# fpgasystems/gcow

Measured on AMD Instinct MI355X. Metric: GiB/s device-resident fp32->ZFP encode, 256Mi-float bucket, 1/2/4/8 GPU, higher is better.
Workload: dtype f32; 1 GPU; c2_1d_fp32_fixed_rate16_256Mi_per_gpu; layout=1-D contiguous, 4-value blocks, mode=fixed-rate, minbits=64, maxbits=64, bucket_bytes_total=1073741824, launcher=none

## Files before the change

### gcow_amd/csrc/enc_fixed1d.hip

```cpp
#include <hip/hip_runtime.h>

#include <algorithm>
#include <stdint.h>

#include "codec_device.h"
#include "field_io.h"
#include "kernels.h"
#include "lean1d.h"
#include "pipe.h"

#ifndef GCOW_C2_U
#define GCOW_C2_U 8
#endif

namespace gcow {

template <int DT>
__device__ __forceinline__ void load_block1d(const void* in, uint64_t nvals, uint32_t b, float* f)
{
  const uint64_t i0 = 4ull * b;
  if (i0 + 4 <= nvals) {
    load_row4<DT>(in, (int64_t)i0, f);
  } else {
    const uint32_t nv = (uint32_t)(nvals - i0);
#pragma unroll
    for (int x = 0; x < 4; x++) f[x] = load_elem<DT>(in, (int64_t)(i0 + pad_index(x, nv)));
  }
}

__device__ __forceinline__ uint32_t spread2_16(uint32_t x)
{
  x = (x | (x << 8)) & 0x00FF00FFu;
  x = (x | (x << 4)) & 0x0F0F0F0Fu;
  x = (x | (x << 2)) & 0x33333333u;
  x = (x | (x << 1)) & 0x55555555u;
  return x;
}

__device__ __forceinline__ uint64_t interleave4_16(uint32_t a, uint32_t b, uint32_t c, uint32_t d)
{
  const uint32_t P = spread2_16(a) | (spread2_16(c) << 1);
  const uint32_t Q = spread2_16(b) | (spread2_16(d) << 1);
  const uint32_t lo = spread2_16(P & 0xffffu) | (spread2_16(Q & 0xffffu) << 1);
  const uint32_t hi = spread2_16(P >> 16) | (spread2_16(Q >> 16) << 1);
  return (uint64_t)lo | ((uint64_t)hi << 32);
}

template <uint32_t WB>
__device__ __forceinline__ uint64_t encode_block1d_fixed(const float* f, const Params& p, const uint16_t* tab)
{
  float fa[4] = {f[0], f[1], f[2], f[3]};
  const int emax = block_emax<4>(fa);
  const uint32_t prec = precision(emax, p.maxprec, p.minexp, 1);
  if (!prec || emax == -127) return 0ull;
  const float s = cast_scale(emax);
  int32_t q[4];
#pragma unroll
  for (int i = 0; i < 4; i++) q[i] = cast1(fa[i], s);
  fwd_lift(q[0], q[1], q[2], q[3]);
  uint32_t u[4];
#pragma unroll
  for (int i = 0; i < 4; i++) u[i] = ((uint32_t)q[i] + 0xaaaaaaaau) ^ 0xaaaaaaaau;
  const int kmin = prec < 32 ? 32 - (int)prec : 0;
  uint64_t acc = 2ull * (uint32_t)(emax + 127) + 1ull;
  uint32_t pos = 9;
  {
    const int L0 = 31 - (int)__builtin_clz(u[0] | 1u) - (u[0] ? 0 : 1);
    const int L1 = 31 - (int)__builtin_clz(u[1] | 1u) - (u[1] ? 0 : 1);
    const int L2 = 31 - (int)__builtin_clz(u[2] | 1u) - (u[2] ? 0 : 1);
    const int L3 = 31 - (int)__builtin_clz(u[3] | 1u) - (u[3] ? 0 : 1);
    const int M0 = max(max(L0, L1), max(L2, L3));
    const int top = max(M0, kmin - 1);
    pos += (uint32_t)(31 - top);
    uint32_t n = 0;
    const int glo = max(L3, kmin);
    for (int k = top; k >= glo && pos < WB; --k) {
      const uint32_t x = ((u[0] >> k) & 1u) | (((u[1] >> k) & 1u) << 1) | (((u[2] >> k) & 1u) << 2) |
                         (((u[3] >> k) & 1u) << 3);
      const uint32_t e = tab[(n << 4) | x];
      acc |= (uint64_t)(e & 127u) << pos;
      pos += (e >> 7) & 7u;
      n = e >> 10;
    }
    const int kt = L3 - 1;
    if (pos < WB && kt >= kmin) {
      const uint32_t sh = (uint32_t)(31 - kt);
      const uint32_t g0 = __builtin_bitreverse32(u[0]) >> sh, g1 = __builtin_bitreverse32(u[1]) >> sh;
      const uint32_t g2 = __builtin_bitreverse32(u[2]) >> sh, g3 = __builtin_bitreverse32(u[3]) >> sh;
      uint64_t J = interleave4_16(g0 & 0xffffu, g1 & 0xffffu, g2 & 0xffffu, g3 & 0xffffu);
      const uint32_t cnt = (uint32_t)(kt - kmin + 1);
      if (cnt < 16) J &= (1ull << (4 * cnt)) - 1ull;
      acc |= J << pos;
    }
  }
  return WB == 64 ? acc : (acc & ((1ull << WB) - 1ull));
}

template <uint32_t WB, bool W2LOW = false>
__device__ __forceinline__ uint64_t encode_block1d_lean6(const float* f, const uint32_t* tab, const uint32_t* rs,
                                                         bool& special)
{
  uint32_t m;
  asm("v_max3_f32 %0, |%1|, |%2|, |%3|" : "=v"(m) : "v"(f[0]), "v"(f[1]), "v"(f[2]));
  asm("v_max_f32_e64 %0, %0, |%1|" : "+v"(m) : "v"(f[3]));
  special = m >= 0x7f800000u || __builtin_isunordered(f[0], f[1]) || __builtin_isunordered(f[2], f[3]);
  const uint32_t E = m >> 23;
  const float s = __uint_as_float((283u - E) << 23);
  uint32_t x = (uint32_t)cvt_i32_hw(f[0] * s), y = (uint32_t)cvt_i32_hw(f[1] * s);
  uint32_t z = (uint32_t)cvt_i32_hw(f[2] * s), w = (uint32_t)cvt_i32_hw(f[3] * s);
  auto asr = [](uint32_t v) { return (uint32_t)((int32_t)v >> 1); };
  constexpr uint32_t NB = 0xaaaaaaaau;
  x = asr(x + w); w -= x;
  z = asr(z + y); y -= z;
  x = asr(x + z); z -= x;
  w = asr(w + y); y -= w;
  const uint32_t u3 = (w + asr(y) + NB) ^ NB;
  const uint32_t u1 = (y - asr(w + asr(y)) + NB) ^ NB;
  const uint32_t u0 = (x + NB) ^ NB, u2 = (z + NB) ^ NB;
  const uint32_t o23 = u2 | u3;
  const uint32_t sh = __builtin_clz(u0 | u1 | o23 | 1u);
  const int M0 = 31 - (int)sh;
  const int jg = (int)min(ffbh_hw(o23), 31u) - (int)sh;
  const uint32_t w0 = u0 << sh, w1 = u1 << sh, w2 = u2 << sh, w3 = u3 << sh;
  const uint64_t Y = window_lds(rs, w0, w1, w2, w3);
  uint32_t pos = 9 + sh;
  uint32_t e = tab[(uint32_t)Y & 255u];
  uint32_t G = e >> 17, gl = (e >> 13) & 15u;
  int j = 4;
  e = tab5_next(tab, e, ((uint32_t)Y >> 8) & 255u);
  G |= (e >> 17) << gl;
  gl += (e >> 13) & 15u;
  const uint32_t hdr = m ? 2u * E + 3u : 0u;
  uint64_t acc = (uint64_t)hdr | ((uint64_t)G << pos);
  pos += gl;
#pragma unroll
  for (int jj = 4; jj < 16; jj += 2) {
    if (j < jj || !__any(jj <= jg)) break;
    e = tab5_next(tab, e, (uint32_t)(Y >> (4 * jj)) & 255u);
    const uint32_t code = pos < WB ? (e >> 17) : 0u;
    acc |= (uint64_t)code << pos;
    pos += (e >> 13) & 15u;
    j = jj + 2;
  }
  const bool tiny = m - 1u < (29u << 23) - 1u;
  special = special || (!tiny && jg >= 16 && pos < WB);
  if (j < 16 && pos < WB) acc |= (Y >> (4 * j)) << pos;
  const uint32_t p2 = pos + 4u * (uint32_t)(16 - j);
  if (__any(p2 < WB && M0 >= 16)) {
    uint64_t Y2;
    if constexpr (W2LOW) {
      Y2 = window_lds_low(rs, w0, w1, w2, w3);
    } else {
      const uint32_t s2 = sh + 16u;
      Y2 = window_lds(rs, u0 << s2, u1 << s2, u2 << s2, u3 << s2);
    }
    if (p2 < WB && M0 >= 16) acc |= Y2 << p2;
  }
  constexpr uint64_t TINY = tiny_payload_cx((int)WB - 9) << 9;
  acc = tiny ? (TINY | hdr) : acc;
  return WB == 64 ? acc : (acc & ((1ull << WB) - 1ull));
}

template <int DT, uint32_t WB, int U, uint32_t T = 256, int V = 0>
__global__ __launch_bounds__(T) void k_encode_fixed1d_np(const void* __restrict__ in, uint32_t nfull, Params p,
                                                         void* __restrict__ out)
{
  __shared__ __attribute__((aligned(16))) uint32_t tab[1280 + 1024];
  constexpr uint32_t IB = DT == DT_BF16 ? 8u : 16u;
  const pipe_v4i rin = buf_rsrc(in, nfull * IB), rout = buf_rsrc(out, nfull * (WB / 8));
  const uint32_t b0 = blockIdx.x * (T * U) + threadIdx.x;
  typename PipeRow<DT>::T r[U];
  if constexpr ((V & 1) != 0) {
    static_assert(T == 256, "table fill assumes 256 threads");
    constexpr int NT = 1280 / 256;
    const pipe_v4i rt = buf_rsrc(&g_plane_tab5, sizeof(PlaneTab2));
    uint32_t tv[NT];
#pragma unroll
    for (int i = 0; i < NT; i++) tv[i] = buf_load_u32((threadIdx.x + 256u * i) * 4u, rt);
#pragma unroll
    for (int k = 0; k < U; k++) r[k] = PipeRow<DT>::load((b0 + T * k) * IB, rin);
#pragma unroll
    for (uint32_t t = threadIdx.x; t < 1024; t += T) tab[1280 + t] = rspread_entry(t);
    asm volatile("s_waitcnt vmcnt(%5)" : "+v"(tv[0]), "+v"(tv[1]), "+v"(tv[2]), "+v"(tv[3]), "+v"(tv[4]) : "n"(U)
                 : "memory");
#pragma unroll
    for (int i = 0; i < NT; i++) tab[threadIdx.x + 256u * i] = tv[i];
  } else {
#pragma unroll
    for (int k = 0; k < U; k++) r[k] = PipeRow<DT>::load((b0 + T * k) * IB, rin);
#pragma unroll
    for (uint32_t t = threadIdx.x; t < 1280; t += T) tab[t] = g_plane_tab5.v[t];
#pragma unroll
    for (uint32_t t = threadIdx.x; t < 1024; t += T) tab[1280 + t] = rspread_entry(t);
  }
  __syncthreads();
#pragma unroll
  for (int k = 0; k < U; k++) {
    pipe_wait<U - 1>(r[k]);
    float f[4];
    PipeRow<DT>::unpack(r[k], f);
    bool special;
    uint64_t w = encode_block1d_lean6<WB, (V & 2) != 0>(f, tab, tab + 1280, special);
    if (special) {
      RegWriter64 rw{0ull, 0u};
      encode_block<1>(rw, f, p);
      w = WB == 64 ? rw.acc : (rw.acc & ((1ull << WB) - 1ull));
    }
    pipe_store<WB>((b0 + T * k) * (WB / 8), rout, w);
  }
}

template <int DT, uint32_t WB, int U>
__global__ __launch_bounds__(256) void k_copy_pattern1d(const void* __restrict__ in, uint32_t nfull,
                                                        void* __restrict__ out)
{
  constexpr uint32_t T = 256;
  constexpr uint32_t IB = DT == DT_BF16 ? 8u : 16u;
  const pipe_v4i rin = buf_rsrc(in, nfull * IB), rout = buf_rsrc(out, nfull * (WB / 8));
  const uint32_t b0 = blockIdx.x * (T * U) + threadIdx.x;
  typename PipeRow<DT>::T r[U];
#pragma unroll
  for (int k = 0; k < U; k++) r[k] = PipeRow<DT>::load((b0 + T * k) * IB, rin);
#pragma unroll
  for (int k = 0; k < U; k++) {
    pipe_wait<U - 1>(r[k]);
    float f[4];
    PipeRow<DT>::unpack(r[k], f);
    const uint64_t w = ((uint64_t)(__float_as_uint(f[0]) ^ __float_as_uint(f[1])) << 32) |
                       (__float_as_uint(f[2]) ^ __float_as_uint(f[3]));
    pipe_store<WB>((b0 + T * k) * (WB / 8), rout, w);
  }
}

template <int DT, uint32_t WB>
__global__ __launch_bounds__(256) void k_encode_fixed1d_generic(const void* __restrict__ in, uint32_t nfull, Params p,
                                                                void* __restrict__ out)
{
  __shared__ uint16_t tab[80];
  if (threadIdx.x < 80) tab[threadIdx.x] = plane_entry4(threadIdx.x);
  __syncthreads();
  constexpr int U = 2;
  const uint32_t b0 = blockIdx.x * (256u * U) + threadIdx.x;
  float f[U][4];
#pragma unroll
  for (int j = 0; j < U; j++) {
    const uint32_t b = b0 + 256u * j;
    if (b < nfull) load_row4<DT>(in, 4ll * b, f[j]);
  }
#pragma unroll
  for (int j = 0; j < U; j++) {
    const uint32_t b = b0 + 256u * j;
    if (b < nfull) {
      const uint64_t w = encode_block1d_fixed<WB>(f[j], p, tab);
      if constexpr (WB == 64) ((uint64_t*)out)[b] = w;
      else ((uint32_t*)out)[b] = (uint32_t)w;
    }
  }
}

template <int DT, uint32_t WB>
__global__ void k_encode_fixed1d_tail(const void* __restrict__ in, uint64_t nvals, uint32_t b, Params p,
                                      void* __restrict__ out)
{
  __shared__ uint16_t tab[80];
  if (threadIdx.x < 80) tab[threadIdx.x] = plane_entry4(threadIdx.x);
  __syncthreads();
  if (threadIdx.x) return;
  float f[4];
  load_block1d<DT>(in, nvals, b, f);
  const uint64_t w = encode_block1d_fixed<WB>(f, p, tab);
  if constexpr (WB == 64) ((uint64_t*)out)[b] = w;
  else ((uint32_t*)out)[b] = (uint32_t)w;
}

static inline hipStream_t S(void* s) { return (hipStream_t)s; }

template <int DT, uint32_t WB>
static void launch_fixed1d_t(const void* in, uint64_t nvals, const Params& p, void* out, hipStream_t st)
{
  const uint32_t nfull = (uint32_t)(nvals / 4);
  if (nfull) {
    const bool kmin0 = p.maxprec >= 32 && p.minexp <= -154;
    if (!kmin0) {
      k_encode_fixed1d_generic<DT, WB><<<(nfull + 511) / 512, 256, 0, st>>>(in, nfull, p, out);
    } else {
      constexpr uint32_t CH = 1u << 27;
      constexpr uint32_t IB = DT == DT_BF16 ? 8u : 16u;
      for (uint32_t c0 = 0; c0 < nfull; c0 += CH) {
        const uint32_t nc = min(CH, nfull - c0);
        const void* ic = (const char*)in + (size_t)c0 * IB;
        void* oc = (char*)out + (size_t)c0 * (WB / 8);
        constexpr int U = GCOW_C2_U;
        k_encode_fixed1d_np<DT, WB, U, 256, 3><<<(nc + 256 * U - 1) / (256 * U), 256, 0, st>>>(ic, nc, p, oc);
      }
    }
  }
  if (nvals % 4) k_encode_fixed1d_tail<DT, WB><<<1, 128, 0, st>>>(in, nvals, nfull, p, out);
}

hipError_t launch_copy_pattern1d(const void* in, int dtype, uint64_t nvals, uint32_t wb, void* out, void* stream)
{
  const uint32_t nfull = (uint32_t)(nvals / 4);
  constexpr uint32_t CH = 1u << 27;
  const uint32_t IB = dtype == DT_BF16 ? 8u : 16u;
  for (uint32_t c0 = 0; c0 < nfull; c0 += CH) {
    const uint32_t nc = std::min(CH, nfull - c0);
    const void* ic = (const char*)in + (size_t)c0 * IB;
    void* oc = (char*)out + (size_t)c0 * (wb / 8);
    const uint32_t g = (nc + 2047) / 2048;
    if (dtype == DT_BF16) {
      if (wb == 64) k_copy_pattern1d<DT_BF16, 64, 8><<<g, 256, 0, S(stream)>>>(ic, nc, oc);
      else k_copy_pattern1d<DT_BF16, 32, 8><<<g, 256, 0, S(stream)>>>(ic, nc, oc);
    } else {
      if (wb == 64) k_copy_pattern1d<DT_F32, 64, 8><<<g, 256, 0, S(stream)>>>(ic, nc, oc);
      else k_copy_pattern1d<DT_F32, 32, 8><<<g, 256, 0, S(stream)>>>(ic, nc, oc);
    }
  }
  return hipGetLastError();
}

hipError_t launch_encode_fixed1d(const void* in, int dtype, uint64_t nvals, uint32_t nblocks, const Params& p,
                                 void* out, void* stream)
{
  (void)nblocks;
  hipStream_t st = S(stream);
  if (dtype == DT_F32) {
    if (p.maxbits == 64) launch_fixed1d_t<DT_F32, 64>(in, nvals, p, out, st);
    else launch_fixed1d_t<DT_F32, 32>(in, nvals, p, out, st);
  } else {
    if (p.maxbits == 64) launch_fixed1d_t<DT_BF16, 64>(in, nvals, p, out, st);
    else launch_fixed1d_t<DT_BF16, 32>(in, nvals, p, out, st);
  }
  return hipGetLastError();
}

}
```

Measured before the change: 3913 GiB/s.

## Micro-optimize lean 1-D fixed-rate encoder instruction selection and special-case path

Reworks the fast 1-D block encoder at the instruction level. It uses v_maximum3 so NaN propagates through the max, packed v2f multiplies for scaling, and LDS lookups with a register-pinned shift constant so addresses fold into shifts. It also adds a branchless header and in-bounds masking, and moves tiny/special classification behind a wave-uniform __any guard. The rspread table fill now computes one entry per thread and stores shifted copies. The aim is fewer VALU instructions per block in a kernel that is largely ALU-bound, at the cost of fragile asm barriers and subtle correctness risk in the rewritten edge cases.

```diff
diff --git a/gcow_amd/csrc/enc_fixed1d.hip b/gcow_amd/csrc/enc_fixed1d.hip
--- a/gcow_amd/csrc/enc_fixed1d.hip
+++ b/gcow_amd/csrc/enc_fixed1d.hip
@@ -96,18 +96,50 @@
   return WB == 64 ? acc : (acc & ((1ull << WB) - 1ull));
 }
 
+__device__ __forceinline__ uint32_t pinned_const(uint32_t c)
+{
+  asm volatile("" : "+v"(c));
+  return c;
+}
+
+__device__ __forceinline__ uint32_t lds_at(const uint32_t* t, uint32_t byte, uint32_t c2)
+{
+  return *(const uint32_t*)((const char*)t + (byte << c2));
+}
+
+__device__ __forceinline__ uint32_t tab5_next_c(const uint32_t* tab, uint32_t e, uint32_t byte, uint32_t c2)
+{
+  uint32_t o = byte << c2;
+  asm("" : "+v"(o));
+  return *(const uint32_t*)((const char*)tab + ((e & 0x1c00u) | o));
+}
+
+template <int LO>
+__device__ __forceinline__ uint64_t window_lds_c(const uint32_t* rs, uint32_t w0, uint32_t w1, uint32_t w2, uint32_t w3,
+                                                 uint32_t c2)
+{
+  constexpr uint32_t A = LO ? 8u : 24u, B = LO ? 0u : 16u;
+  const uint32_t lo = lds_at(rs, (w0 >> A) & 255u, c2) | lds_at(rs + 256, (w1 >> A) & 255u, c2) |
+                      lds_at(rs + 512, (w2 >> A) & 255u, c2) | lds_at(rs + 768, (w3 >> A) & 255u, c2);
+  const uint32_t hi = lds_at(rs, (w0 >> B) & 255u, c2) | lds_at(rs + 256, (w1 >> B) & 255u, c2) |
+                      lds_at(rs + 512, (w2 >> B) & 255u, c2) | lds_at(rs + 768, (w3 >> B) & 255u, c2);
+  return (uint64_t)lo | ((uint64_t)hi << 32);
+}
+
 template <uint32_t WB, bool W2LOW = false>
 __device__ __forceinline__ uint64_t encode_block1d_lean6(const float* f, const uint32_t* tab, const uint32_t* rs,
-                                                         bool& special)
+                                                         bool& special, uint32_t c2 = 2u, uint32_t c0 = 0u)
 {
   uint32_t m;
-  asm("v_max3_f32 %0, |%1|, |%2|, |%3|" : "=v"(m) : "v"(f[0]), "v"(f[1]), "v"(f[2]));
-  asm("v_max_f32_e64 %0, %0, |%1|" : "+v"(m) : "v"(f[3]));
-  special = m >= 0x7f800000u || __builtin_isunordered(f[0], f[1]) || __builtin_isunordered(f[2], f[3]);
-  const uint32_t E = m >> 23;
+  asm("v_maximum3_f32 %0, |%1|, |%2|, |%3|" : "=v"(m) : "v"(f[0]), "v"(f[1]), "v"(f[2]));
+  asm("v_maximum3_f32 %0, %0, |%1|, |%1|" : "+v"(m) : "v"(f[3]));
+  uint32_t E = m >> 23;
+  asm("" : "+v"(E));
   const float s = __uint_as_float((283u - E) << 23);
-  uint32_t x = (uint32_t)cvt_i32_hw(f[0] * s), y = (uint32_t)cvt_i32_hw(f[1] * s);
-  uint32_t z = (uint32_t)cvt_i32_hw(f[2] * s), w = (uint32_t)cvt_i32_hw(f[3] * s);
+  typedef float v2f __attribute__((ext_vector_type(2)));
+  const v2f p01 = v2f{f[0], f[1]} * s, p23 = v2f{f[2], f[3]} * s;
+  uint32_t x = (uint32_t)cvt_i32_hw(p01.x), y = (uint32_t)cvt_i32_hw(p01.y);
+  uint32_t z = (uint32_t)cvt_i32_hw(p23.x), w = (uint32_t)cvt_i32_hw(p23.y);
   auto asr = [](uint32_t v) { return (uint32_t)((int32_t)v >> 1); };
   constexpr uint32_t NB = 0xaaaaaaaau;
   x = asr(x + w); w -= x;
@@ -122,43 +154,74 @@
   const int M0 = 31 - (int)sh;
   const int jg = (int)min(ffbh_hw(o23), 31u) - (int)sh;
   const uint32_t w0 = u0 << sh, w1 = u1 << sh, w2 = u2 << sh, w3 = u3 << sh;
-  const uint64_t Y = window_lds(rs, w0, w1, w2, w3);
+  uint64_t Y = window_lds_c<0>(rs, w0, w1, w2, w3, c2);
+  {
+    uint32_t ylo = (uint32_t)Y;
+    asm("" : "+v"(ylo));
+    Y = (Y & 0xffffffff00000000ull) | ylo;
+  }
   uint32_t pos = 9 + sh;
-  uint32_t e = tab[(uint32_t)Y & 255u];
+  uint32_t e = lds_at(tab, (uint32_t)Y & 255u, c2);
   uint32_t G = e >> 17, gl = (e >> 13) & 15u;
   int j = 4;
-  e = tab5_next(tab, e, ((uint32_t)Y >> 8) & 255u);
+  e = tab5_next_c(tab, e, ((uint32_t)Y >> 8) & 255u, c2);
   G |= (e >> 17) << gl;
   gl += (e >> 13) & 15u;
-  const uint32_t hdr = m ? 2u * E + 3u : 0u;
-  uint64_t acc = (uint64_t)hdr | ((uint64_t)G << pos);
+  const uint32_t hdr = (E << 1) + min(m, 3u);
+  uint64_t acc = (uint64_t)hdr | (((uint64_t)G | ((uint64_t)c0 << 32)) << pos);
   pos += gl;
 #pragma unroll
   for (int jj = 4; jj < 16; jj += 2) {
     if (j < jj || !__any(jj <= jg)) break;
-    e = tab5_next(tab, e, (uint32_t)(Y >> (4 * jj)) & 255u);
+    e = tab5_next_c(tab, e, (uint32_t)(Y >> (4 * jj)) & 255u, c2);
     const uint32_t code = pos < WB ? (e >> 17) : 0u;
-    acc |= (uint64_t)code << pos;
+    acc |= ((uint64_t)code | ((uint64_t)c0 << 32)) << pos;
     pos += (e >> 13) & 15u;
     j = jj + 2;
   }
-  const bool tiny = m - 1u < (29u << 23) - 1u;
-  special = special || (!tiny && jg >= 16 && pos < WB);
-  if (j < 16 && pos < WB) acc |= (Y >> (4 * j)) << pos;
-  const uint32_t p2 = pos + 4u * (uint32_t)(16 - j);
-  if (__any(p2 < WB && M0 >= 16)) {
-    uint64_t Y2;
-    if constexpr (W2LOW) {
-      Y2 = window_lds_low(rs, w0, w1, w2, w3);
-    } else {
+  const bool past = jg >= 16 && pos < WB;
+  uint32_t inb = pos < WB ? ~0u : 0u;
+  asm("" : "+v"(inb));
+  if (j < 16) {
+    const uint64_t V = (Y >> (4 * j)) << pos;
+    acc = (uint64_t)(((uint32_t)V & inb) | (uint32_t)acc) |
+          ((uint64_t)(((uint32_t)(V >> 32) & inb) | (uint32_t)(acc >> 32)) << 32);
+  }
+  const uint32_t p2 = pos - 4u * (uint32_t)j;
+  if constexpr (W2LOW) {
+    if (__any(pos + (64u - WB) < 4u * (uint32_t)j)) {
+      const uint64_t Y2 = window_lds_c<1>(rs, w0, w1, w2, w3, c2);
+      if (pos + (64u - WB) < 4u * (uint32_t)j) acc |= Y2 << (p2 & 63u);
+    }
+  } else {
+    if (__any(pos + (64u - WB) < 4u * (uint32_t)j && M0 >= 16)) {
       const uint32_t s2 = sh + 16u;
-      Y2 = window_lds(rs, u0 << s2, u1 << s2, u2 << s2, u3 << s2);
-    }
-    if (p2 < WB && M0 >= 16) acc |= Y2 << p2;
-  }
-  constexpr uint64_t TINY = tiny_payload_cx((int)WB - 9) << 9;
-  acc = tiny ? (TINY | hdr) : acc;
+      const uint64_t Y2 = window_lds(rs, u0 << s2, u1 << s2, u2 << s2, u3 << s2);
+      if (pos + (64u - WB) < 4u * (uint32_t)j && M0 >= 16) acc |= Y2 << (p2 & 63u);
+    }
+  }
+  constexpr uint32_t TLO = 29u << 23, INF = 0x7f800000u;
+  special = past;
+  if (__any(m - TLO >= INF - TLO && m != 0u)) {
+    constexpr uint64_t TINY = tiny_payload_cx((int)WB - 9) << 9;
+    const bool tiny = m - 1u < TLO - 1u;
+    special = m >= INF || (!tiny && past);
+    acc = tiny ? (TINY | max(hdr, 3u)) : acc;
+  }
   return WB == 64 ? acc : (acc & ((1ull << WB) - 1ull));
+}
+
+template <uint32_t T>
+__device__ __forceinline__ void fill_rspread(uint32_t* rs)
+{
+  if constexpr (T == 256) {
+    const uint32_t b = threadIdx.x & 255u, v = rspread_entry(b);
+#pragma unroll
+    for (uint32_t i = 0; i < 4; i++) rs[256 * i + b] = v << i;
+  } else {
+#pragma unroll
+    for (uint32_t t = threadIdx.x; t < 1024; t += T) rs[t] = rspread_entry(t);
+  }
 }
 
 template <int DT, uint32_t WB, int U, uint32_t T = 256, int V = 0>
@@ -179,8 +242,7 @@
     for (int i = 0; i < NT; i++) tv[i] = buf_load_u32((threadIdx.x + 256u * i) * 4u, rt);
 #pragma unroll
     for (int k = 0; k < U; k++) r[k] = PipeRow<DT>::load((b0 + T * k) * IB, rin);
-#pragma unroll
-    for (uint32_t t = threadIdx.x; t < 1024; t += T) tab[1280 + t] = rspread_entry(t);
+    fill_rspread<T>(tab + 1280);
     asm volatile("s_waitcnt vmcnt(%5)" : "+v"(tv[0]), "+v"(tv[1]), "+v"(tv[2]), "+v"(tv[3]), "+v"(tv[4]) : "n"(U)
                  : "memory");
 #pragma unroll
@@ -190,17 +252,17 @@
     for (int k = 0; k < U; k++) r[k] = PipeRow<DT>::load((b0 + T * k) * IB, rin);
 #pragma unroll
     for (uint32_t t = threadIdx.x; t < 1280; t += T) tab[t] = g_plane_tab5.v[t];
-#pragma unroll
-    for (uint32_t t = threadIdx.x; t < 1024; t += T) tab[1280 + t] = rspread_entry(t);
+    fill_rspread<T>(tab + 1280);
   }
   __syncthreads();
+  const uint32_t c2 = pinned_const(2u), c0 = pinned_const(0u);
 #pragma unroll
   for (int k = 0; k < U; k++) {
     pipe_wait<U - 1>(r[k]);
     float f[4];
     PipeRow<DT>::unpack(r[k], f);
     bool special;
-    uint64_t w = encode_block1d_lean6<WB, (V & 2) != 0>(f, tab, tab + 1280, special);
+    uint64_t w = encode_block1d_lean6<WB, (V & 2) != 0>(f, tab, tab + 1280, special, c2, c0);
     if (special) {
       RegWriter64 rw{0ull, 0u};
       encode_block<1>(rw, f, p);
```

Result: no change. 3928 GiB/s (median of 6 runs) (+0.4%).

## Add straight-line fast-path encoder with deferred odd-block fallback pass

Applied to the files above, without the earlier changes.

Introduces a branch-light fast-path 1-D block encoder that handles common blocks and flags odd cases (out of range, NaN, tiny, overflow of the plane budget). Flagged blocks have their store redirected to an out-of-range offset and are re-encoded afterwards in a second loop using the old lean6/general encoder. The shared-memory plane table is now loaded with 128-bit buffer loads instead of 32-bit loads. The aim is to cut per-block divergence and instruction count in the main loop, at the cost of re-unpacking rows and keeping the input registers live longer for the fallback.

```diff
diff --git a/gcow_amd/csrc/enc_fixed1d.hip b/gcow_amd/csrc/enc_fixed1d.hip
--- a/gcow_amd/csrc/enc_fixed1d.hip
+++ b/gcow_amd/csrc/enc_fixed1d.hip
@@ -161,52 +161,134 @@
   return WB == 64 ? acc : (acc & ((1ull << WB) - 1ull));
 }
 
-template <int DT, uint32_t WB, int U, uint32_t T = 256, int V = 0>
+template <uint32_t WB>
+__device__ __forceinline__ uint64_t encode_block1d_straight(const float* f, const uint32_t* tab, const uint32_t* rs,
+                                                            bool& odd)
+{
+  typedef float v2f __attribute__((ext_vector_type(2)));
+  uint32_t m;
+  asm("v_max3_f32 %0, |%1|, |%2|, |%3|" : "=v"(m) : "v"(f[0]), "v"(f[1]), "v"(f[2]));
+  asm("v_max_f32_e64 %0, %0, |%1|" : "+v"(m) : "v"(f[3]));
+  const uint32_t E = m >> 23;
+  const float s = __uint_as_float((283u - E) << 23);
+  const v2f s2 = {s, s};
+  const v2f p01 = (v2f){f[0], f[1]} * s2, p23 = (v2f){f[2], f[3]} * s2;
+  uint32_t x = (uint32_t)cvt_i32_hw(p01.x), y = (uint32_t)cvt_i32_hw(p01.y);
+  uint32_t z = (uint32_t)cvt_i32_hw(p23.x), w = (uint32_t)cvt_i32_hw(p23.y);
+  auto asr = [](uint32_t v) { return (uint32_t)((int32_t)v >> 1); };
+  constexpr uint32_t NB = 0xaaaaaaaau;
+  x = asr(x + w); w -= x;
+  z = asr(z + y); y -= z;
+  x = asr(x + z); z -= x;
+  w = asr(w + y); y -= w;
+  const uint32_t u3 = (w + asr(y) + NB) ^ NB;
+  const uint32_t u1 = (y - asr(w + asr(y)) + NB) ^ NB;
+  const uint32_t u0 = (x + NB) ^ NB, u2 = (z + NB) ^ NB;
+  const uint32_t o23 = u2 | u3;
+  const uint32_t sh = __builtin_clz(u0 | u1 | o23 | 1u);
+  const int jg = (int)min(ffbh_hw(o23), 31u) - (int)sh;
+  const uint64_t Y = window_lds(rs, u0 << sh, u1 << sh, u2 << sh, u3 << sh);
+  uint32_t pos = 9 + sh;
+  constexpr int J0 = 4, JCAP = 16;
+  uint32_t e = tab[(uint32_t)Y & 255u];
+  uint32_t G = e >> 17, gl = (e >> 13) & 15u;
+  e = tab5_next(tab, e, ((uint32_t)Y >> 8) & 255u);
+  G |= (e >> 17) << gl;
+  gl += (e >> 13) & 15u;
+  uint64_t acc = (uint64_t)min(m, 2u * E + 3u) | ((uint64_t)G << pos);
+  pos += gl;
+  int j = J0;
+  bool far = false;
+#pragma unroll
+  for (int jj = J0; jj < JCAP; jj += 2) {
+    if (j < jj || !__any(jj <= jg)) break;
+    e = tab5_next(tab, e, (uint32_t)(Y >> (4 * jj)) & 255u);
+    acc |= (uint64_t)(e >> 17) << (pos & 63u);
+    pos += (e >> 13) & 15u;
+    j = jj + 2;
+    if (j >= JCAP) far = jg >= JCAP;
+  }
+  if (j < 16) acc |= (Y >> (4 * j)) << (pos & 63u);
+  const bool range = m - (29u << 23) >= (0x7f800000u - (29u << 23)) && m != 0u;
+  odd = range || __builtin_isunordered(f[0], f[1]) || __builtin_isunordered(f[2], f[3]) || far || pos >= 64u ||
+        pos + (64u - WB) < 4u * (uint32_t)j;
+  return WB == 64 ? acc : (acc & ((1ull << WB) - 1ull));
+}
+
+template <uint32_t WB>
+__device__ __forceinline__ bool tiny_block1d(const float* f, uint64_t& w)
+{
+  uint32_t m;
+  asm("v_max3_f32 %0, |%1|, |%2|, |%3|" : "=v"(m) : "v"(f[0]), "v"(f[1]), "v"(f[2]));
+  asm("v_max_f32_e64 %0, %0, |%1|" : "+v"(m) : "v"(f[3]));
+  const bool tiny = m - 1u < (29u << 23) - 1u && !__builtin_isunordered(f[0], f[1]) && !__builtin_isunordered(f[2], f[3]);
+  constexpr uint64_t TINY = (tiny_payload_cx((int)WB - 9) << 9) & (WB == 64 ? ~0ull : (1ull << (WB & 63u)) - 1ull);
+  w = tiny ? (TINY | (2u * (m >> 23) + 3u)) : w;
+  return tiny;
+}
+
+constexpr uint32_t kDropOffset = 0x80000000u;
+
+template <int DT, uint32_t WB, int U, uint32_t T = 256>
 __global__ __launch_bounds__(T) void k_encode_fixed1d_np(const void* __restrict__ in, uint32_t nfull, Params p,
                                                          void* __restrict__ out)
 {
-  __shared__ __attribute__((aligned(16))) uint32_t tab[1280 + 1024];
+  constexpr uint32_t NTAB = 1280;
+  __shared__ __attribute__((aligned(16))) uint32_t tab[NTAB + 1024];
   constexpr uint32_t IB = DT == DT_BF16 ? 8u : 16u;
   const pipe_v4i rin = buf_rsrc(in, nfull * IB), rout = buf_rsrc(out, nfull * (WB / 8));
   const uint32_t b0 = blockIdx.x * (T * U) + threadIdx.x;
   typename PipeRow<DT>::T r[U];
-  if constexpr ((V & 1) != 0) {
-    static_assert(T == 256, "table fill assumes 256 threads");
-    constexpr int NT = 1280 / 256;
+  {
+    constexpr uint32_t TCH = NTAB / 4, TR = (TCH + T - 1) / T;
     const pipe_v4i rt = buf_rsrc(&g_plane_tab5, sizeof(PlaneTab2));
-    uint32_t tv[NT];
-#pragma unroll
-    for (int i = 0; i < NT; i++) tv[i] = buf_load_u32((threadIdx.x + 256u * i) * 4u, rt);
+    pipe_v4u tv[TR];
+#pragma unroll
+    for (uint32_t i = 0; i < TR; i++) tv[i] = buf_load_b128((threadIdx.x + T * i) * 16u, rt);
 #pragma unroll
     for (int k = 0; k < U; k++) r[k] = PipeRow<DT>::load((b0 + T * k) * IB, rin);
 #pragma unroll
-    for (uint32_t t = threadIdx.x; t < 1024; t += T) tab[1280 + t] = rspread_entry(t);
-    asm volatile("s_waitcnt vmcnt(%5)" : "+v"(tv[0]), "+v"(tv[1]), "+v"(tv[2]), "+v"(tv[3]), "+v"(tv[4]) : "n"(U)
-                 : "memory");
-#pragma unroll
-    for (int i = 0; i < NT; i++) tab[threadIdx.x + 256u * i] = tv[i];
-  } else {
-#pragma unroll
-    for (int k = 0; k < U; k++) r[k] = PipeRow<DT>::load((b0 + T * k) * IB, rin);
-#pragma unroll
-    for (uint32_t t = threadIdx.x; t < 1280; t += T) tab[t] = g_plane_tab5.v[t];
-#pragma unroll
-    for (uint32_t t = threadIdx.x; t < 1024; t += T) tab[1280 + t] = rspread_entry(t);
+    for (uint32_t t = 0; t < 1024; t += T)
+      if (t + T <= 1024 || threadIdx.x < 1024 - t) tab[NTAB + t + threadIdx.x] = rspread_entry(t + threadIdx.x);
+    asm volatile("s_waitcnt vmcnt(%0)" : : "n"(U) : "memory");
+#pragma unroll
+    for (uint32_t i = 0; i < TR; i++) asm volatile("" : "+v"(tv[i]));
+#pragma unroll
+    for (uint32_t i = 0; i < TR; i++)
+      if (T * (i + 1) <= TCH || threadIdx.x + T * i < TCH) ((pipe_v4u*)tab)[threadIdx.x + T * i] = tv[i];
   }
   __syncthreads();
+  uint32_t oddm = 0;
 #pragma unroll
   for (int k = 0; k < U; k++) {
     pipe_wait<U - 1>(r[k]);
     float f[4];
     PipeRow<DT>::unpack(r[k], f);
+    bool odd;
+    uint64_t w = encode_block1d_straight<WB>(f, tab, tab + NTAB, odd);
+    uint32_t off = (b0 + T * k) * (WB / 8);
+    if (__any(odd)) {
+      odd = odd && !tiny_block1d<WB>(f, w);
+      oddm |= odd ? 1u << k : 0u;
+      off = odd ? kDropOffset : off;
+    }
+    pipe_store<WB>(off, rout, w);
+  }
+  if (!__any(oddm != 0u)) return;
+#pragma unroll
+  for (int k = 0; k < U; k++) {
+    const bool mine = (oddm >> k) & 1u;
+    if (!__any(mine)) continue;
+    float f[4];
+    PipeRow<DT>::unpack(r[k], f);
     bool special;
-    uint64_t w = encode_block1d_lean6<WB, (V & 2) != 0>(f, tab, tab + 1280, special);
+    uint64_t w = encode_block1d_lean6<WB, true>(f, tab, tab + NTAB, special);
     if (special) {
       RegWriter64 rw{0ull, 0u};
       encode_block<1>(rw, f, p);
       w = WB == 64 ? rw.acc : (rw.acc & ((1ull << WB) - 1ull));
     }
-    pipe_store<WB>((b0 + T * k) * (WB / 8), rout, w);
+    pipe_store<WB>(mine ? (b0 + T * k) * (WB / 8) : kDropOffset, rout, w);
   }
 }
 
@@ -291,7 +373,7 @@
         const void* ic = (const char*)in + (size_t)c0 * IB;
         void* oc = (char*)out + (size_t)c0 * (WB / 8);
         constexpr int U = GCOW_C2_U;
-        k_encode_fixed1d_np<DT, WB, U, 256, 3><<<(nc + 256 * U - 1) / (256 * U), 256, 0, st>>>(ic, nc, p, oc);
+        k_encode_fixed1d_np<DT, WB, U><<<(nc + 256 * U - 1) / (256 * U), 256, 0, st>>>(ic, nc, p, oc);
       }
     }
   }
```

Result: no change. 3912 GiB/s before, 3917 GiB/s after, median of 3 (+0.1%).
